# snakers4/mnasnet-pytorch

Measured on AMD Instinct MI355X. Metric: images/sec MNASNet-1.0 224^2 bf16 train step, higher is better.
Workload: dtype bf16

## Files before the change

mnasnet_pytorch_amd/csrc/mnas_pws.hip:

```cpp
#include "mnas_common.h"
#ifndef MNAS_PWS_D2
#define MNAS_PWS_D2 1
#endif

struct PwsArgs {
    int M, K, N;
    int Kpad, ksteps;
    int n_pad16;
    MnasActIn act;
    MnasGradIn grad;
    const uint16_t* w;
    const float* bias;
    const void* resid;
    void* out;
    float* stats;
    const void* red_y;
    const float* red_bn;
    const float* gate;
    int hw;
};

template <int MODE, int NT, int KSW, int NW, bool GATE = false>
__global__ __launch_bounds__(64 * NW) void k_pws(PwsArgs a) {
    static_assert(!GATE || MODE == 0, "the gate is an act-on-load extension of the forward");
    extern __shared__ __attribute__((aligned(16))) unsigned char smem[];
    constexpr int NB = NT * 16, CROWS = MODE == 1 ? 5 : 2;
    constexpr int PP = NB + 4;
    constexpr int NTH = 64 * NW;
    float* lds_coef = (float*)smem;
    float* lds_part = lds_coef + CROWS * a.Kpad;
    float* lds_redc = lds_part + 2 * NW * 16 * PP;
    float* lds_fin = lds_part;

    const int tid = threadIdx.x, lane = tid & 63, wave = tid >> 6;
    const int l15 = lane & 15, lg = lane >> 4;
    const int n0 = blockIdx.y * NB;
    const int nb_valid = min(NB, a.N - n0);
    const int chunks = nb_valid >> 3;
    const bool has_coef = MODE == 1 || a.act.scale != nullptr;
    const bool do_red = MODE == 1 && a.red_y != nullptr;

    const int ngroups = (a.M + 15) >> 4;
    uint4 v0[KSW], v1[MODE == 1 ? KSW : 1];
    constexpr bool D2 = MNAS_PWS_D2 && !GATE && MODE == 1;
    uint4 w0[D2 ? KSW : 1], w1[(D2 && MODE == 1) ? KSW : 1];
    float gq[GATE ? KSW : 1][8];
    auto issue_to = [&](int g, uint4* d0, uint4* d1) {
        const int m = g * 16 + l15;
#pragma unroll
        for (int j = 0; j < KSW; ++j) {
            const int k = (wave + NW * j) * 32 + lg * 8;
            d0[j] = make_uint4(0, 0, 0, 0);
            if (MODE == 1) d1[j] = make_uint4(0, 0, 0, 0);
            if (m < a.M && k < a.K) {
                const size_t off = (size_t)m * a.K + k;
                if (MODE == 0) d0[j] = *(const uint4*)((const uint16_t*)a.act.data + off);
                else {
                    d0[j] = *(const uint4*)((const uint16_t*)a.grad.g + off);
                    d1[j] = *(const uint4*)((const uint16_t*)a.grad.y + off);
                }
            }
        }
    };
    auto issue = [&](int g) {
        const int m = g * 16 + l15;
        const float* grow = GATE ? a.gate + (size_t)(m / a.hw) * a.K : nullptr;
#pragma unroll
        for (int j = 0; j < KSW; ++j) {
            const int k = (wave + NW * j) * 32 + lg * 8;
            v0[j] = make_uint4(0, 0, 0, 0);
            if (MODE == 1) v1[j] = make_uint4(0, 0, 0, 0);
            if (m < a.M && k < a.K) {
                const size_t off = (size_t)m * a.K + k;
                if constexpr (GATE) {
                    const float4 a0 = *(const float4*)(grow + k), a1 = *(const float4*)(grow + k + 4);
                    gq[j][0] = a0.x; gq[j][1] = a0.y; gq[j][2] = a0.z; gq[j][3] = a0.w;
                    gq[j][4] = a1.x; gq[j][5] = a1.y; gq[j][6] = a1.z; gq[j][7] = a1.w;
                }
                if (MODE == 0) v0[j] = *(const uint4*)((const uint16_t*)a.act.data + off);
                else {
                    v0[j] = *(const uint4*)((const uint16_t*)a.grad.g + off);
                    v1[j] = *(const uint4*)((const uint16_t*)a.grad.y + off);
                }
            }
        }
    };
    int it = 0;
    auto first_issue = [&]() {
        if ((int)blockIdx.x < ngroups) { if constexpr (D2) issue_to(blockIdx.x, v0, v1); else issue(blockIdx.x); }
        if constexpr (D2) { if ((int)(blockIdx.x + gridDim.x) < ngroups) issue_to(blockIdx.x + gridDim.x, w0, w1); }
    };
    if (MNAS_EARLY) first_issue();
    bf16x8_t wf[NT][KSW];
#pragma unroll
    for (int j = 0; j < KSW; ++j) {
        const int ks = wave + NW * j;
#pragma unroll
        for (int nt = 0; nt < NT; ++nt) {
            const int row = n0 + nt * 16 + l15;
            uint4 v = make_uint4(0, 0, 0, 0);
            if (ks < a.ksteps && row < a.n_pad16) v = *(const uint4*)(a.w + (size_t)row * a.Kpad + ks * 32 + lg * 8);
            wf[nt][j] = *(const bf16x8_t*)&v;
        }
    }
    mnas_fill_table(lds_coef, CROWS * a.Kpad, tid, NTH, [&](int i) {
        const int r = i / a.Kpad, c = i - r * a.Kpad;
        float v = 0.f;
        if (c < a.K) {
            if (MODE == 1) v = a.grad.coef[(size_t)r * a.K + c];
            else if (has_coef) v = r == 0 ? a.act.scale[c] : a.act.shift[c];
        }
        return v;
    });
    if (do_red)
        mnas_fill_table(lds_redc, 4 * NB, tid, NTH, [&](int i) {
            const int r = i / NB, co = n0 + i % NB;
            return co < a.N ? mnas_red_coef(a.red_bn, a.N, r, co) : 0.f;
        });
    __syncthreads();
    if (!MNAS_EARLY) first_issue();

    const bool epi = tid < 16 * chunks;
    const int ep = epi ? tid / chunks : 0, ec8 = epi ? tid - ep * chunks : 0;
    float bias8[8], s1[8], s2[8];
#pragma unroll
    for (int j = 0; j < 8; ++j) {
        bias8[j] = (MODE == 0 && epi && a.bias) ? a.bias[n0 + ec8 * 8 + j] : 0.f;
        s1[j] = 0.f; s2[j] = 0.f;
    }

    for (int g = blockIdx.x; g < ngroups; g += gridDim.x, ++it) {
        const int m0 = g * 16;
        bf16x8_t bf[KSW];
#pragma unroll
        for (int j = 0; j < KSW; ++j) {
            const int k = (wave + NW * j) * 32 + lg * 8;
            uint4 v = v0[j];
            if (has_coef && k < a.K && m0 + l15 < a.M) {
                float cf[CROWS][8];
#pragma unroll
                for (int r = 0; r < CROWS; ++r) {
                    *(float4*)&cf[r][0] = *(const float4*)(lds_coef + r * a.Kpad + k);
                    *(float4*)&cf[r][4] = *(const float4*)(lds_coef + r * a.Kpad + k + 4);
                }
                if (MODE == 0) {
                    if constexpr (GATE) v = act8g(v, cf[0], cf[1], gq[j]);
                    else v = act8(v, cf[0], cf[1]);
                } else {
                    float o[8];
                    dy8(v, v1[j], cf[0], cf[1], cf[2 % CROWS], cf[3 % CROWS], cf[4 % CROWS], o);
                    v = pack8(o);
                }
            }
            bf[j] = *(const bf16x8_t*)&v;
        }
        uint4 rpre = make_uint4(0, 0, 0, 0), ypre = make_uint4(0, 0, 0, 0);
        if (MODE == 1 && epi && m0 + ep < a.M) {
            const size_t o = (size_t)(m0 + ep) * a.N + n0 + ec8 * 8;
            if (a.resid) rpre = *(const uint4*)((const uint16_t*)a.resid + o);
            if (do_red) ypre = *(const uint4*)((const uint16_t*)a.red_y + o);
        }
        if constexpr (D2) {
#pragma unroll
            for (int j = 0; j < KSW; ++j) { v0[j] = w0[j]; if (MODE == 1) v1[j] = w1[j]; }
            if (g + 2 * (int)gridDim.x < ngroups) issue_to(g + 2 * gridDim.x, w0, w1);
        } else if (g + (int)gridDim.x < ngroups) issue(g + gridDim.x);
        f32x4_t acc[NT];
#pragma unroll
        for (int nt = 0; nt < NT; ++nt) acc[nt] = (f32x4_t){0.f, 0.f, 0.f, 0.f};
#pragma unroll
        for (int j = 0; j < KSW; ++j)
#pragma unroll
            for (int nt = 0; nt < NT; ++nt) acc[nt] = __builtin_amdgcn_mfma_f32_16x16x32_bf16(wf[nt][j], bf[j], acc[nt], 0, 0, 0);
        float* part = lds_part + ((it & 1) * NW + wave) * 16 * PP + l15 * PP + lg * 4;
#pragma unroll
        for (int nt = 0; nt < NT; ++nt) *(float4*)(part + nt * 16) = *(const float4*)&acc[nt];
        __syncthreads();
        if (epi && m0 + ep < a.M) {
            float v[8];
            const float* src = lds_part + (it & 1) * NW * 16 * PP + ep * PP + ec8 * 8;
            *(float4*)&v[0] = *(const float4*)src;
            *(float4*)&v[4] = *(const float4*)(src + 4);
#pragma unroll
            for (int w = 1; w < NW; ++w) {
                const float4 x0 = *(const float4*)(src + w * 16 * PP), x1 = *(const float4*)(src + w * 16 * PP + 4);
                v[0] += x0.x; v[1] += x0.y; v[2] += x0.z; v[3] += x0.w;
                v[4] += x1.x; v[5] += x1.y; v[6] += x1.z; v[7] += x1.w;
            }
            const size_t o = (size_t)(m0 + ep) * a.N + n0 + ec8 * 8;
            if (MODE == 0) {
#pragma unroll
                for (int j = 0; j < 4; ++j) {
                    const mnas_f2 w2 = mnas_ld2(v + 2 * j) + mnas_ld2(bias8 + 2 * j);
                    v[2 * j] = w2.x; v[2 * j + 1] = w2.y;
                    mnas_stat2(w2, s1 + 2 * j, s2 + 2 * j);
                }
                *(uint4*)((uint16_t*)a.out + o) = pack8(v);
            } else {
                if (a.resid) {
                    float r[8];
                    unpack8(rpre, r);
#pragma unroll
                    for (int j = 0; j < 8; ++j) v[j] += r[j];
                }
                const uint4 pk = pack8(v);
                *(uint4*)((uint16_t*)a.out + o) = pk;
                if (do_red) {
                    const uint32_t gu[4] = {pk.x, pk.y, pk.z, pk.w}, yu[4] = {ypre.x, ypre.y, ypre.z, ypre.w};
                    const int cl = ec8 * 8;
#pragma unroll
                    for (int j = 0; j < 4; ++j)
                        mnas_red2(gu[j], yu[j], mnas_ld2(lds_redc + cl + 2 * j), mnas_ld2(lds_redc + NB + cl + 2 * j),
                                  mnas_ld2(lds_redc + 2 * NB + cl + 2 * j), mnas_ld2(lds_redc + 3 * NB + cl + 2 * j), s1 + 2 * j, s2 + 2 * j);
                }
            }
        }
    }
    if ((MODE == 0 || do_red) && a.stats) {
        __syncthreads();
        if (epi) {
#pragma unroll
            for (int j = 0; j < 8; ++j) {
                lds_fin[(ep * 2 + 0) * NB + ec8 * 8 + j] = s1[j];
                lds_fin[(ep * 2 + 1) * NB + ec8 * 8 + j] = s2[j];
            }
        }
        __syncthreads();
        for (int i = tid; i < 2 * nb_valid; i += NTH) {
            const int r = i / nb_valid, cl = i - r * nb_valid;
            float v = lds_fin[r * NB + cl];
            for (int p = 1; p < 16; ++p) v += lds_fin[(p * 2 + r) * NB + cl];
            a.stats[((size_t)r * a.N + n0 + cl) * gridDim.x + blockIdx.x] = v;
        }
    }
}

struct PwsPlan { int nt, ksw, nw, nblocks; size_t lds; };
static bool pws_plan(int mode, int M, int K, int N, PwsPlan* p) {
    if ((K & 7) || (N & 7) || K < 192 || N < 8 || M < 1) return false;
    if (mode == 1 && mnas_pws_enabled() < 2) return false;
    if (M > 250000) return false;
    const int ksteps = (K + 31) / 32;
    const int tiles = (N + 15) / 16;
    int nt = tiles <= 3 ? 3 : 6;
    const int nblocks = (tiles + nt - 1) / nt;
    if (nblocks * nt - tiles > 3) return false;
    const int nw = (ksteps > 20 || (mode == 1 && ksteps >= 12)) ? 8 : 4;
    const int ksw_need = (ksteps + nw - 1) / nw;
    if (ksw_need > (mode == 1 ? 3 : 5)) return false;
    p->nt = nt; p->nw = nw; p->ksw = ksw_need <= 2 ? 2 : (ksw_need == 3 ? 3 : 5); p->nblocks = nblocks;
    const int NB = nt * 16, Kpad = ksteps * 32, crows = mode == 1 ? 5 : 2;
    size_t part = (size_t)2 * nw * 16 * (NB + 4) * 4, fin = (size_t)16 * 2 * NB * 4;
    p->lds = (size_t)crows * Kpad * 4 + (part > fin ? part : fin) + (size_t)4 * NB * 4;
    return p->lds <= 160 * 1024;
}
int mnas_pws_parts(int mode, int M, int K, int N) {
    PwsPlan p;
    if (!mnas_pws_enabled() || !pws_plan(mode, M, K, N, &p)) return -1;
    const int ngroups = (M + 15) / 16;
    const int base = mnas_diag_env("MNAS_PWS_WGS", 512);
    int want = base / p.nblocks;
    if (p.nw == 8) want = base / 2 / p.nblocks;
    if (want < 32) want = 32;
    return ngroups < want ? ngroups : want;
}

template <int MODE, int NT, int KSW, int NW>
static int pws_launch(const PwsArgs& a, const PwsPlan& p, int nparts, hipStream_t s) {
    if (a.gate) {
        if constexpr (MODE == 0 && KSW <= 3) {
            hipLaunchKernelGGL((k_pws<MODE, NT, KSW, NW, true>), dim3(nparts, p.nblocks), dim3(64 * NW), p.lds, s, a);
            MNAS_CHECK_LAUNCH();
            return MNAS_OK;
        }
        return MNAS_EINVAL;
    }
    hipLaunchKernelGGL((k_pws<MODE, NT, KSW, NW>), dim3(nparts, p.nblocks), dim3(64 * NW), p.lds, s, a);
    MNAS_CHECK_LAUNCH();
    return MNAS_OK;
}
template <int MODE>
static int pws_dispatch(const PwsArgs& a, const PwsPlan& p, int nparts, hipStream_t s) {
#define MNAS_PWS(NT_, KSW_, NW_) if (p.nt == NT_ && p.ksw == KSW_ && p.nw == NW_) return pws_launch<MODE, NT_, KSW_, NW_>(a, p, nparts, s);
    MNAS_PWS(3, 2, 4) MNAS_PWS(3, 5, 4) MNAS_PWS(6, 2, 4) MNAS_PWS(6, 5, 4) MNAS_PWS(3, 5, 8) MNAS_PWS(6, 5, 8)
    MNAS_PWS(3, 2, 8) MNAS_PWS(6, 2, 8) MNAS_PWS(3, 3, 8) MNAS_PWS(6, 3, 8) MNAS_PWS(3, 3, 4) MNAS_PWS(6, 3, 4)
#undef MNAS_PWS
    return MNAS_EINVAL;
}

int mnas_pws_gate_ok(int M, int K, int N) {
    PwsPlan p;
    return (mnas_pws_enabled() && pws_plan(0, M, K, N, &p) && p.ksw <= 3) ? 1 : 0;
}

int mnas_pws_accepts(const MnasConvGemm* c) {
    const int M = c->N * c->Ho * c->Wo;
    PwsPlan p;
    if (!pws_plan(c->mode, M, c->Ci, c->Co, &p) || (c->mode == 1 && !c->grad.coef)) return 0;
    if (c->mode == 0 && c->gate && (!c->act.scale || p.ksw > 3)) return 0;
    return 1;
}
int mnas_pws_run(const MnasConvGemm* c, void* stream) {
    const int M = c->N * c->Ho * c->Wo;
    PwsPlan p;
    if (!mnas_pws_accepts(c) || !pws_plan(c->mode, M, c->Ci, c->Co, &p)) return MNAS_EINVAL;
    PwsArgs a;
    a.M = M; a.K = c->Ci; a.N = c->Co;
    a.ksteps = (c->Ci + 31) / 32; a.Kpad = a.ksteps * 32;
    a.n_pad16 = (c->Co + 15) / 16 * 16;
    a.act = c->act; a.grad = c->grad; a.w = (const uint16_t*)c->w; a.bias = c->bias; a.resid = c->resid; a.out = c->out;
    a.stats = c->stats; a.red_y = c->mode == 1 ? c->red_y : nullptr; a.red_bn = c->red_bn;
    a.gate = c->mode == 0 ? c->gate : nullptr; a.hw = c->Ho * c->Wo;
    if (a.gate && (!c->act.scale || p.ksw > 3)) return MNAS_EINVAL;
    hipStream_t s = (hipStream_t)stream;
    return c->mode == 0 ? pws_dispatch<0>(a, p, c->nparts, s) : pws_dispatch<1>(a, p, c->nparts, s);
}
```

Before: 26160.

## Restructure pointwise GEMM prefetch into two-buffer ping-pong with unguarded clamped loads

Replaces the register-copy double prefetch (D2) in the backward pointwise kernel with a loop unrolled by two that alternates between two register buffers, removing the per-iteration copy of prefetched tiles. Global loads now clamp row and k indices rather than branching, so loads are issued unconditionally and masking happens at consume time. An empty asm barrier keeps the weight fragments in registers. This trades some redundant out-of-range loads and extra register pressure for fewer moves and branches in the hot loop.

```diff
diff --git a/mnasnet_pytorch_amd/csrc/mnas_pws.hip b/mnasnet_pytorch_amd/csrc/mnas_pws.hip
--- a/mnasnet_pytorch_amd/csrc/mnas_pws.hip
+++ b/mnasnet_pytorch_amd/csrc/mnas_pws.hip
@@ -1,6 +1,6 @@
 #include "mnas_common.h"
-#ifndef MNAS_PWS_D2
-#define MNAS_PWS_D2 1
+#ifndef MNAS_PWS_AHEAD2
+#define MNAS_PWS_AHEAD2 1
 #endif
 
 struct PwsArgs {
@@ -20,9 +20,10 @@
     int hw;
 };
 
-template <int MODE, int NT, int KSW, int NW, bool GATE = false>
+template <int MODE, int NT, int KSW, int NW, bool GATE = false, bool AHEAD2 = false>
 __global__ __launch_bounds__(64 * NW) void k_pws(PwsArgs a) {
     static_assert(!GATE || MODE == 0, "the gate is an act-on-load extension of the forward");
+    static_assert(!(GATE && AHEAD2), "the gated forms load one group ahead");
     extern __shared__ __attribute__((aligned(16))) unsigned char smem[];
     constexpr int NB = NT * 16, CROWS = MODE == 1 ? 5 : 2;
     constexpr int PP = NB + 4;
@@ -41,54 +42,33 @@
     const bool do_red = MODE == 1 && a.red_y != nullptr;
 
     const int ngroups = (a.M + 15) >> 4;
+    const int G = gridDim.x;
     uint4 v0[KSW], v1[MODE == 1 ? KSW : 1];
-    constexpr bool D2 = MNAS_PWS_D2 && !GATE && MODE == 1;
-    uint4 w0[D2 ? KSW : 1], w1[(D2 && MODE == 1) ? KSW : 1];
+    uint4 u0[AHEAD2 ? KSW : 1], u1[(AHEAD2 && MODE == 1) ? KSW : 1];
     float gq[GATE ? KSW : 1][8];
-    auto issue_to = [&](int g, uint4* d0, uint4* d1) {
-        const int m = g * 16 + l15;
+    auto issue = [&](int g, uint4* d0, uint4* d1) {
+        const int m = min(g * 16 + l15, a.M - 1);
+        const float* grow = GATE ? a.gate + (size_t)(m / a.hw) * a.K : nullptr;
 #pragma unroll
         for (int j = 0; j < KSW; ++j) {
-            const int k = (wave + NW * j) * 32 + lg * 8;
-            d0[j] = make_uint4(0, 0, 0, 0);
-            if (MODE == 1) d1[j] = make_uint4(0, 0, 0, 0);
-            if (m < a.M && k < a.K) {
-                const size_t off = (size_t)m * a.K + k;
-                if (MODE == 0) d0[j] = *(const uint4*)((const uint16_t*)a.act.data + off);
-                else {
-                    d0[j] = *(const uint4*)((const uint16_t*)a.grad.g + off);
-                    d1[j] = *(const uint4*)((const uint16_t*)a.grad.y + off);
-                }
-            }
-        }
-    };
-    auto issue = [&](int g) {
-        const int m = g * 16 + l15;
-        const float* grow = GATE ? a.gate + (size_t)(m / a.hw) * a.K : nullptr;
-#pragma unroll
-        for (int j = 0; j < KSW; ++j) {
-            const int k = (wave + NW * j) * 32 + lg * 8;
-            v0[j] = make_uint4(0, 0, 0, 0);
-            if (MODE == 1) v1[j] = make_uint4(0, 0, 0, 0);
-            if (m < a.M && k < a.K) {
-                const size_t off = (size_t)m * a.K + k;
-                if constexpr (GATE) {
-                    const float4 a0 = *(const float4*)(grow + k), a1 = *(const float4*)(grow + k + 4);
-                    gq[j][0] = a0.x; gq[j][1] = a0.y; gq[j][2] = a0.z; gq[j][3] = a0.w;
-                    gq[j][4] = a1.x; gq[j][5] = a1.y; gq[j][6] = a1.z; gq[j][7] = a1.w;
-                }
-                if (MODE == 0) v0[j] = *(const uint4*)((const uint16_t*)a.act.data + off);
-                else {
-                    v0[j] = *(const uint4*)((const uint16_t*)a.grad.g + off);
-                    v1[j] = *(const uint4*)((const uint16_t*)a.grad.y + off);
-                }
-            }
-        }
-    };
-    int it = 0;
+            const int k0 = (wave + NW * j) * 32 + lg * 8;
+            const int k = k0 < a.K ? k0 : 0;
+            const size_t off = (size_t)m * a.K + k;
+            if constexpr (GATE) {
+                const float4 a0 = *(const float4*)(grow + k), a1 = *(const float4*)(grow + k + 4);
+                gq[j][0] = a0.x; gq[j][1] = a0.y; gq[j][2] = a0.z; gq[j][3] = a0.w;
+                gq[j][4] = a1.x; gq[j][5] = a1.y; gq[j][6] = a1.z; gq[j][7] = a1.w;
+            }
+            if (MODE == 0) d0[j] = *(const uint4*)((const uint16_t*)a.act.data + off);
+            else {
+                d0[j] = *(const uint4*)((const uint16_t*)a.grad.g + off);
+                d1[j] = *(const uint4*)((const uint16_t*)a.grad.y + off);
+            }
+        }
+    };
     auto first_issue = [&]() {
-        if ((int)blockIdx.x < ngroups) { if constexpr (D2) issue_to(blockIdx.x, v0, v1); else issue(blockIdx.x); }
-        if constexpr (D2) { if ((int)(blockIdx.x + gridDim.x) < ngroups) issue_to(blockIdx.x + gridDim.x, w0, w1); }
+        issue(blockIdx.x, v0, v1);
+        if constexpr (AHEAD2) issue(blockIdx.x + G, u0, u1);
     };
     if (MNAS_EARLY) first_issue();
     bf16x8_t wf[NT][KSW];
@@ -119,6 +99,10 @@
         });
     __syncthreads();
     if (!MNAS_EARLY) first_issue();
+#pragma unroll
+    for (int j = 0; j < KSW; ++j)
+#pragma unroll
+        for (int nt = 0; nt < NT; ++nt) asm volatile("" ::"v"(wf[nt][j]));
 
     const bool epi = tid < 16 * chunks;
     const int ep = epi ? tid / chunks : 0, ec8 = epi ? tid - ep * chunks : 0;
@@ -128,57 +112,43 @@
         bias8[j] = (MODE == 0 && epi && a.bias) ? a.bias[n0 + ec8 * 8 + j] : 0.f;
         s1[j] = 0.f; s2[j] = 0.f;
     }
-
-    for (int g = blockIdx.x; g < ngroups; g += gridDim.x, ++it) {
-        const int m0 = g * 16;
-        bf16x8_t bf[KSW];
-#pragma unroll
-        for (int j = 0; j < KSW; ++j) {
-            const int k = (wave + NW * j) * 32 + lg * 8;
-            uint4 v = v0[j];
-            if (has_coef && k < a.K && m0 + l15 < a.M) {
-                float cf[CROWS][8];
-#pragma unroll
-                for (int r = 0; r < CROWS; ++r) {
-                    *(float4*)&cf[r][0] = *(const float4*)(lds_coef + r * a.Kpad + k);
-                    *(float4*)&cf[r][4] = *(const float4*)(lds_coef + r * a.Kpad + k + 4);
-                }
-                if (MODE == 0) {
-                    if constexpr (GATE) v = act8g(v, cf[0], cf[1], gq[j]);
-                    else v = act8(v, cf[0], cf[1]);
-                } else {
-                    float o[8];
-                    dy8(v, v1[j], cf[0], cf[1], cf[2 % CROWS], cf[3 % CROWS], cf[4 % CROWS], o);
-                    v = pack8(o);
-                }
-            }
-            bf[j] = *(const bf16x8_t*)&v;
-        }
-        uint4 rpre = make_uint4(0, 0, 0, 0), ypre = make_uint4(0, 0, 0, 0);
+    auto xform = [&](uint4 v, int j, int m0, const float (*cf)[8], const uint4* y) {
+        if (m0 + l15 < a.M) {
+            if (MODE == 0) {
+                if constexpr (GATE) v = act8g(v, cf[0], cf[1], gq[j]);
+                else v = act8(v, cf[0], cf[1]);
+            } else {
+                float o[8];
+                dy8(v, y[j], cf[0], cf[1], cf[2 % CROWS], cf[3 % CROWS], cf[4 % CROWS], o);
+                v = pack8(o);
+            }
+        }
+        return v;
+    };
+    auto load_coef = [&](int k, float (*cf)[8]) {
+#pragma unroll
+        for (int r = 0; r < CROWS; ++r) {
+            *(float4*)&cf[r][0] = *(const float4*)(lds_coef + r * a.Kpad + k);
+            *(float4*)&cf[r][4] = *(const float4*)(lds_coef + r * a.Kpad + k + 4);
+        }
+    };
+    auto epi_issue = [&](int m0, uint4& rpre, uint4& ypre) {
+        rpre = make_uint4(0, 0, 0, 0); ypre = make_uint4(0, 0, 0, 0);
         if (MODE == 1 && epi && m0 + ep < a.M) {
             const size_t o = (size_t)(m0 + ep) * a.N + n0 + ec8 * 8;
             if (a.resid) rpre = *(const uint4*)((const uint16_t*)a.resid + o);
             if (do_red) ypre = *(const uint4*)((const uint16_t*)a.red_y + o);
         }
-        if constexpr (D2) {
-#pragma unroll
-            for (int j = 0; j < KSW; ++j) { v0[j] = w0[j]; if (MODE == 1) v1[j] = w1[j]; }
-            if (g + 2 * (int)gridDim.x < ngroups) issue_to(g + 2 * gridDim.x, w0, w1);
-        } else if (g + (int)gridDim.x < ngroups) issue(g + gridDim.x);
-        f32x4_t acc[NT];
-#pragma unroll
-        for (int nt = 0; nt < NT; ++nt) acc[nt] = (f32x4_t){0.f, 0.f, 0.f, 0.f};
-#pragma unroll
-        for (int j = 0; j < KSW; ++j)
-#pragma unroll
-            for (int nt = 0; nt < NT; ++nt) acc[nt] = __builtin_amdgcn_mfma_f32_16x16x32_bf16(wf[nt][j], bf[j], acc[nt], 0, 0, 0);
-        float* part = lds_part + ((it & 1) * NW + wave) * 16 * PP + l15 * PP + lg * 4;
+    };
+    auto park = [&](int buf, const f32x4_t* acc) {
+        float* part = lds_part + (buf * NW + wave) * 16 * PP + l15 * PP + lg * 4;
 #pragma unroll
         for (int nt = 0; nt < NT; ++nt) *(float4*)(part + nt * 16) = *(const float4*)&acc[nt];
-        __syncthreads();
+    };
+    auto epilogue = [&](int buf, int m0, const uint4& rpre, const uint4& ypre) {
         if (epi && m0 + ep < a.M) {
             float v[8];
-            const float* src = lds_part + (it & 1) * NW * 16 * PP + ep * PP + ec8 * 8;
+            const float* src = lds_part + buf * NW * 16 * PP + ep * PP + ec8 * 8;
             *(float4*)&v[0] = *(const float4*)src;
             *(float4*)&v[4] = *(const float4*)(src + 4);
 #pragma unroll
@@ -215,6 +185,45 @@
                 }
             }
         }
+    };
+
+    int g = blockIdx.x;
+    auto one = [&](int g1, uint4* d0, uint4* d1, int buf, int gnext) {
+        const int m0 = g1 * 16;
+        bf16x8_t bf[KSW];
+#pragma unroll
+        for (int j = 0; j < KSW; ++j) {
+            const int k = (wave + NW * j) * 32 + lg * 8;
+            uint4 v = k < a.K ? d0[j] : make_uint4(0, 0, 0, 0);
+            if (has_coef && k < a.K && m0 + l15 < a.M) {
+                float cf[CROWS][8];
+                load_coef(k, cf);
+                v = xform(v, j, m0, cf, d1);
+            }
+            bf[j] = *(const bf16x8_t*)&v;
+        }
+        uint4 rpre, ypre;
+        epi_issue(m0, rpre, ypre);
+        issue(gnext, d0, d1);
+        f32x4_t acc[NT];
+#pragma unroll
+        for (int nt = 0; nt < NT; ++nt) acc[nt] = (f32x4_t){0.f, 0.f, 0.f, 0.f};
+#pragma unroll
+        for (int j = 0; j < KSW; ++j)
+#pragma unroll
+            for (int nt = 0; nt < NT; ++nt) acc[nt] = __builtin_amdgcn_mfma_f32_16x16x32_bf16(wf[nt][j], bf[j], acc[nt], 0, 0, 0);
+        park(buf, acc);
+        __syncthreads();
+        epilogue(buf, m0, rpre, ypre);
+    };
+    if constexpr (AHEAD2) {
+        for (; g + G < ngroups; g += 2 * G) {
+            one(g, v0, v1, 0, g + 2 * G);
+            one(g + G, u0, u1, 1, g + 3 * G);
+        }
+        if (g < ngroups) one(g, v0, v1, 0, ngroups);
+    } else {
+        for (int it = 0; g < ngroups; g += G, ++it) one(g, v0, v1, it & 1, g + G);
     }
     if ((MODE == 0 || do_red) && a.stats) {
         __syncthreads();
@@ -235,7 +244,8 @@
     }
 }
 
-struct PwsPlan { int nt, ksw, nw, nblocks; size_t lds; };
+struct PwsPlan { int nt, ksw, nw, nblocks; bool ahead2; size_t lds; };
+static constexpr bool pws_ahead2(int mode, int ksw) { return MNAS_PWS_AHEAD2 && mode == 1 && ksw <= 3; }
 static bool pws_plan(int mode, int M, int K, int N, PwsPlan* p) {
     if ((K & 7) || (N & 7) || K < 192 || N < 8 || M < 1) return false;
     if (mode == 1 && mnas_pws_enabled() < 2) return false;
@@ -249,6 +259,7 @@
     const int ksw_need = (ksteps + nw - 1) / nw;
     if (ksw_need > (mode == 1 ? 3 : 5)) return false;
     p->nt = nt; p->nw = nw; p->ksw = ksw_need <= 2 ? 2 : (ksw_need == 3 ? 3 : 5); p->nblocks = nblocks;
+    p->ahead2 = pws_ahead2(mode, p->ksw);
     const int NB = nt * 16, Kpad = ksteps * 32, crows = mode == 1 ? 5 : 2;
     size_t part = (size_t)2 * nw * 16 * (NB + 4) * 4, fin = (size_t)16 * 2 * NB * 4;
     p->lds = (size_t)crows * Kpad * 4 + (part > fin ? part : fin) + (size_t)4 * NB * 4;
@@ -275,7 +286,9 @@
         }
         return MNAS_EINVAL;
     }
-    hipLaunchKernelGGL((k_pws<MODE, NT, KSW, NW>), dim3(nparts, p.nblocks), dim3(64 * NW), p.lds, s, a);
+    constexpr bool AHEAD2 = pws_ahead2(MODE, KSW);
+    if (p.ahead2 != AHEAD2) return MNAS_EINVAL;
+    hipLaunchKernelGGL((k_pws<MODE, NT, KSW, NW, false, AHEAD2>), dim3(nparts, p.nblocks), dim3(64 * NW), p.lds, s, a);
     MNAS_CHECK_LAUNCH();
     return MNAS_OK;
 }
```

After: 26210, median of 5. Within noise of the previous version (+0.2%).
